# YihongSun/Dynamo-Depth

Hardware: AMD Instinct MI355X
Metric: training images/sec (192x640 triplets) (higher is better)
Workload: dtype f32

## Files before the change

dynamo-depth_amd/csrc/dd_conv_mfma.hip:

```cpp
#include <hip/hip_runtime.h>
#include <cstdlib>
#include <type_traits>

#include "../../include/dynamo_hip.h"
#include "dd_attr.h"
#include "dd_split.h"
#include "dd_store_tile.h"

namespace dd {
namespace cm {

constexpr int TH = 8, TW = 32, NT = 256;
constexpr int HH = TH + 2, HW = TW + 2, HN = HH * HW;
constexpr int CK = 16;
constexpr int PSTR = 48;
constexpr int A_PIECE = HN * PSTR;
constexpr int A_BYTES = 3 * A_PIECE;
__device__ __forceinline__ int halo_addr(int px, int half) {
  return px * 48 + half * 16;
}
__host__ __device__ constexpr int pieces_of(int products) { return products == 6 ? 3 : (products == 3 ? 2 : 1); }
constexpr int FRAG = 1024;
constexpr int PRE = (HN * 4 + NT - 1) / NT;

__host__ __device__ inline int blocks_for(int n_out) { return n_out <= 32 ? 1 : (n_out <= 64 ? 2 : (n_out <= 96 ? 3 : 2)); }
__host__ __device__ inline int frags_of(int n_out, int k_in) {
  const int NB = blocks_for(n_out);
  return ((n_out + 32 * NB - 1) / (32 * NB)) * ((k_in + CK - 1) / CK) * 9 * NB;
}

template <int NB>
constexpr int b_buf_bytes() { return ((3 * NB + 3) / 4) * 4 * FRAG; }

template <int NB>
constexpr int lds_bytes() { return A_BYTES + 2 * b_buf_bytes<NB>(); }

__device__ __forceinline__ void pack_fragment(const float* __restrict__ w, long long s_co, long long s_ci, long long s_kh, long long s_kw, int cout, int cin,
                                              uint4* __restrict__ pack_fwd, uint4* __restrict__ pack_bwd, int frags_fwd, int frags_bwd, int gid) {
  const int lane = gid & 63;
  int f = gid >> 6;
  const bool bwd = f >= frags_fwd;
  if (bwd) f -= frags_fwd;
  if (bwd ? (f >= frags_bwd || !pack_bwd) : !pack_fwd) return;
  const int n_out = bwd ? cin : cout, k_in = bwd ? cout : cin;
  const int nchunks = (k_in + CK - 1) / CK, NB = blocks_for(n_out);
  const int blk = f % NB, tap = (f / NB) % 9, chunk = (f / (NB * 9)) % nchunks, tile = f / (NB * 9 * nchunks);
  const int o = (tile * NB + blk) * 32 + (lane & 31);
  const int i0 = chunk * CK + (lane >> 5) * 8;
  const int kh = tap / 3, kw = tap % 3;
  float v[8];
#pragma unroll
  for (int e = 0; e < 8; ++e) {
    const int i = i0 + e;
    float val = 0.f;
    if (o < n_out && i < k_in)
      val = bwd ? w[(long long)i * s_co + (long long)o * s_ci + (2 - kh) * s_kh + (2 - kw) * s_kw]
                : w[(long long)o * s_co + (long long)i * s_ci + kh * s_kh + kw * s_kw];
    v[e] = val;
  }
  unsigned p[3][4];
#pragma unroll
  for (int q = 0; q < 4; ++q) split2(v[2 * q], v[2 * q + 1], p[0][q], p[1][q], p[2][q]);
  uint4* dst = (bwd ? pack_bwd : pack_fwd) + ((size_t)f * 3) * 64 + lane;
#pragma unroll
  for (int pc = 0; pc < 3; ++pc) dst[pc * 64] = make_uint4(p[pc][0], p[pc][1], p[pc][2], p[pc][3]);
}

__global__ __launch_bounds__(256) void conv_mfma_pack_kernel(const float* __restrict__ w, long long s_co, long long s_ci, long long s_kh, long long s_kw,
                                                             int cout, int cin, uint4* __restrict__ pack_fwd, uint4* __restrict__ pack_bwd,
                                                             int frags_fwd, int frags_bwd) {
  pack_fragment(w, s_co, s_ci, s_kh, s_kw, cout, cin, pack_fwd, pack_bwd, frags_fwd, frags_bwd, blockIdx.x * 256 + threadIdx.x);
}

constexpr int PACK_JOB_WORDS = 10;
__global__ __launch_bounds__(256) void conv_mfma_pack_many_kernel(const long long* __restrict__ jobs, const int* __restrict__ block_job) {
  const long long* j = jobs + (size_t)block_job[blockIdx.x] * PACK_JOB_WORDS;
  const int cout = (int)j[5], cin = (int)j[6];
  uint4* const pf = reinterpret_cast<uint4*>(j[7]);
  uint4* const pb = reinterpret_cast<uint4*>(j[8]);
  const int frags_fwd = pf ? frags_of(cout, cin) : 0, frags_bwd = pb ? frags_of(cin, cout) : 0;
  pack_fragment(reinterpret_cast<const float*>(j[0]), j[1], j[2], j[3], j[4], cout, cin, pf, pb, frags_fwd, frags_bwd,
                (blockIdx.x - (int)j[9]) * 256 + threadIdx.x);
}

template <int NB, int NP>
__global__ __launch_bounds__(NT, 2) void conv_mfma_kernel(const float* __restrict__ x, const uint4* __restrict__ pack, const float* __restrict__ bias,
                                                          int Hi, int Wi, int Ho, int Wo, int k_in, int n_out, int pad, int tiles_x, int tiles_y,
                                                          float* __restrict__ y) {
  extern __shared__ __align__(16) unsigned char smem[];
  unsigned char* const s_b = smem + A_BYTES;
  const int tid = threadIdx.x, lane = tid & 63, wave = __builtin_amdgcn_readfirstlane(tid >> 6);
  const int b = blockIdx.z, ntile = blockIdx.y;
  int tile = blockIdx.x;
  {
    const int ntiles = gridDim.x, xc = tile & 7, base = ntiles >> 3, extra = ntiles & 7;
    tile = xc * base + min(xc, extra) + (tile >> 3);
  }
  const int X0 = (tile % tiles_x) * TW, Y0 = (tile / tiles_x) * TH;
  const int nchunks = (k_in + CK - 1) / CK;
  const float* xb = x + (size_t)b * Hi * Wi * k_in;
  const char* pk = reinterpret_cast<const char*>(pack) + (size_t)ntile * nchunks * 9 * (3 * NB * FRAG);

  int g_off[PRE];
  int l_off[PRE];
#pragma unroll
  for (int j = 0; j < PRE; ++j) {
    const int i = tid + j * NT, px = i >> 2, q = i & 3;
    const int hy = px / HW, hx = px - hy * HW;
    const int Y = Y0 - pad + hy, X = X0 - pad + hx;
    l_off[j] = px < HN ? halo_addr(px, q >> 1) + (q & 1) * 8 : -1;
    g_off[j] = (px < HN && Y >= 0 && Y < Hi && X >= 0 && X < Wi) ? (Y * Wi + X) * k_in + q * 4 : -1;
  }
  float4 pre[PRE];
  auto fetch = [&](int chunk) {
#pragma unroll
    for (int j = 0; j < PRE; ++j) {
      const int c0 = chunk * CK + (((tid + j * NT) & 3) << 2);
      const int off = (g_off[j] >= 0 && c0 < k_in) ? g_off[j] + chunk * CK : 0;
      pre[j] = *reinterpret_cast<const float4*>(xb + off);
    }
  };
  auto stage = [&](int chunk) {
#pragma unroll
    for (int j = 0; j < PRE; ++j) {
      if (l_off[j] >= 0) {
        const int c0 = chunk * CK + (((tid + j * NT) & 3) << 2);
        const bool in = g_off[j] >= 0 && c0 < k_in;
        const float4 v = in ? pre[j] : make_float4(0.f, 0.f, 0.f, 0.f);
        unsigned a1, a2, a3, b1, b2, b3;
        split2(v.x, v.y, a1, a2, a3);
        split2(v.z, v.w, b1, b2, b3);
        *reinterpret_cast<uint2*>(smem + l_off[j]) = make_uint2(a1, b1);
        if (pieces_of(NP) > 1) *reinterpret_cast<uint2*>(smem + A_PIECE + l_off[j]) = make_uint2(a2, b2);
        if (pieces_of(NP) > 2) *reinterpret_cast<uint2*>(smem + 2 * A_PIECE + l_off[j]) = make_uint2(a3, b3);
      }
    }
  };
  constexpr int BR = (3 * NB + 3) / 4;
  uint4 breg[BR];
#pragma unroll
  for (int r = 0; r < BR; ++r) breg[r] = make_uint4(0u, 0u, 0u, 0u);
  auto fetch_b = [&](int s) {
    const char* src = pk + (size_t)s * (3 * NB * FRAG) + lane * 16;
#pragma unroll
    for (int r = 0; r < BR; ++r)
      breg[r] = *reinterpret_cast<const uint4*>(src + (wave + 4 * r < 3 * NB ? wave + 4 * r : 0) * FRAG);
  };
  auto store_b = [&](int s) {
    unsigned char* dst = s_b + (s & 1) * b_buf_bytes<NB>() + lane * 16;
#pragma unroll
    for (int r = 0; r < BR; ++r) *reinterpret_cast<uint4*>(dst + (wave + 4 * r) * FRAG) = breg[r];
  };
  auto lds_barrier = [&]() { asm volatile("s_waitcnt lgkmcnt(0)\n\ts_barrier" ::: "memory"); };

  f16v acc[2][NB];
#pragma unroll
  for (int m = 0; m < 2; ++m)
#pragma unroll
    for (int n = 0; n < NB; ++n)
#pragma unroll
      for (int r = 0; r < 16; ++r) acc[m][n][r] = 0.f;

  const int a_pix = (2 * wave) * HW + (lane & 31), a_half = lane >> 5;
  const unsigned char* b_lane = s_b + lane * 16;

  uint4 af[2][2][3], bfr[2][NB][3];
  auto read_frags = [&](int set, int tap, int s) {
    const int ty = tap / 3, tx = tap % 3;
#pragma unroll
    for (int m = 0; m < 2; ++m) {
      const unsigned char* ap = smem + halo_addr(a_pix + (m + ty) * HW + tx, a_half);
#pragma unroll
      for (int pc = 0; pc < pieces_of(NP); ++pc) af[set][m][pc] = *reinterpret_cast<const uint4*>(ap + pc * A_PIECE);
    }
    const unsigned char* bb = b_lane + (s & 1) * b_buf_bytes<NB>();
#pragma unroll
    for (int n = 0; n < NB; ++n)
#pragma unroll
      for (int pc = 0; pc < pieces_of(NP); ++pc) bfr[set][n][pc] = *reinterpret_cast<const uint4*>(bb + (n * 3 + pc) * FRAG);
  };

  const int nsteps = nchunks * 9;
  float bv[NB];
#pragma unroll
  for (int n = 0; n < NB; ++n) bv[n] = tile_bias(bias, (ntile * NB + n) * 32 + (lane & 31), n_out, pack);
  fetch_b(0);
  fetch(0);
  store_b(0);
  fetch_b(1);
  for (int chunk = 0; chunk < nchunks; ++chunk) {
    lds_barrier();
    stage(chunk);
    store_b(chunk * 9 + 1);
    lds_barrier();
    read_frags(0, 0, chunk * 9);
#pragma unroll
    for (int tap = 0; tap < 9; ++tap) {
      const int s = chunk * 9 + tap, cur = tap & 1;
      if (tap < 8) read_frags(cur ^ 1, tap + 1, s + 1);
      fetch_b(min(s + 2, nsteps - 1));
      if (tap == 1) fetch(min(chunk + 1, nchunks - 1));
      constexpr int PA[6] = {2, 0, 1, 1, 0, 0}, PB[6] = {0, 2, 1, 0, 1, 0};
#pragma unroll
      for (int t = 6 - NP; t < 6; ++t)
#pragma unroll
        for (int m = 0; m < 2; ++m)
#pragma unroll
          for (int n = 0; n < NB; ++n)
            acc[m][n] = __builtin_amdgcn_mfma_f32_32x32x16_bf16(__builtin_bit_cast(bf8, af[cur][m][PA[t]]), __builtin_bit_cast(bf8, bfr[cur][n][PB[t]]), acc[m][n], 0, 0, 0);
      __builtin_amdgcn_sched_barrier(0);
      if (tap < 8) {
        store_b(s + 2);
        lds_barrier();
      }
    }
  }

  auto tail = [&](auto full) {
#pragma unroll
    for (int n = 0; n < NB; ++n) {
      const int co = (ntile * NB + n) * 32 + (lane & 31);
#pragma unroll
      for (int m = 0; m < 2; ++m) {
        const int Y = Y0 + 2 * wave + m, X = X0 + 4 * (lane >> 5);
        float* p = y + (((size_t)b * Ho + Y) * Wo + X) * n_out + co;
        store_acc32<decltype(full)::value>(acc[m][n], bv[n], p, (size_t)n_out, (co < n_out && Y < Ho) ? Wo - X : 0, StoreF32{});
      }
    }
  };
  if (X0 + TW <= Wo && Y0 + TH <= Ho && (ntile + 1) * (32 * NB) <= n_out) tail(std::true_type{});
  else tail(std::false_type{});
}

constexpr int FLAT_MT = 256;
constexpr int FLAT_ZERO = HN - 1;
constexpr int FLAT_MAX_W = (FLAT_ZERO - FLAT_MT) / 2 - 1;

template <int NB, int NP>
__global__ __launch_bounds__(NT, 2) void conv_mfma_flat_kernel(const float* __restrict__ x, const uint4* __restrict__ pack, const float* __restrict__ bias,
                                                               int H, int W, int M, int k_in, int n_out, int splits, float* __restrict__ out) {
  extern __shared__ __align__(16) unsigned char smem[];
  unsigned char* const s_b = smem + A_BYTES;
  const int tid = threadIdx.x, lane = tid & 63, wave = __builtin_amdgcn_readfirstlane(tid >> 6);
  const int p0 = (int)blockIdx.x * FLAT_MT, ntile = blockIdx.y, split = blockIdx.z;
  const int nchunks = (k_in + CK - 1) / CK;
  const int c_begin = (int)((long long)nchunks * split / splits), c_end = (int)((long long)nchunks * (split + 1) / splits);
  const int win = FLAT_MT + 2 * (W + 1), q0 = p0 - (W + 1);
  const char* pk = reinterpret_cast<const char*>(pack) + (size_t)ntile * nchunks * 9 * (3 * NB * FRAG);

  int g_off[PRE], l_off[PRE];
#pragma unroll
  for (int j = 0; j < PRE; ++j) {
    const int i = tid + j * NT, px = i >> 2, q = i & 3;
    const int fp = q0 + px;
    l_off[j] = px < win ? halo_addr(px, q >> 1) + (q & 1) * 8 : -1;
    g_off[j] = (px < win && fp >= 0 && fp < M) ? fp * k_in + q * 4 : -1;
  }
  if (tid < 9) {
    const int pc = tid / 3, part = tid % 3;
    if (part * 16 < PSTR) *reinterpret_cast<uint4*>(smem + pc * A_PIECE + FLAT_ZERO * PSTR + part * 16) = make_uint4(0u, 0u, 0u, 0u);
  }
  float4 pre[PRE];
  auto fetch = [&](int chunk) {
#pragma unroll
    for (int j = 0; j < PRE; ++j) {
      const int c0 = chunk * CK + (((tid + j * NT) & 3) << 2);
      const int off = (g_off[j] >= 0 && c0 < k_in) ? g_off[j] + chunk * CK : 0;
      pre[j] = *reinterpret_cast<const float4*>(x + off);
    }
  };
  auto stage = [&](int chunk) {
#pragma unroll
    for (int j = 0; j < PRE; ++j) {
      if (l_off[j] >= 0) {
        const int c0 = chunk * CK + (((tid + j * NT) & 3) << 2);
        const bool in = g_off[j] >= 0 && c0 < k_in;
        const float4 v = in ? pre[j] : make_float4(0.f, 0.f, 0.f, 0.f);
        unsigned a1, a2, a3, b1, b2, b3;
        split2(v.x, v.y, a1, a2, a3);
        split2(v.z, v.w, b1, b2, b3);
        *reinterpret_cast<uint2*>(smem + l_off[j]) = make_uint2(a1, b1);
        if (pieces_of(NP) > 1) *reinterpret_cast<uint2*>(smem + A_PIECE + l_off[j]) = make_uint2(a2, b2);
        if (pieces_of(NP) > 2) *reinterpret_cast<uint2*>(smem + 2 * A_PIECE + l_off[j]) = make_uint2(a3, b3);
      }
    }
  };
  constexpr int BR = (3 * NB + 3) / 4;
  uint4 breg[BR];
#pragma unroll
  for (int r = 0; r < BR; ++r) breg[r] = make_uint4(0u, 0u, 0u, 0u);
  auto fetch_b = [&](int s) {
    const char* src = pk + (size_t)s * (3 * NB * FRAG) + lane * 16;
#pragma unroll
    for (int r = 0; r < BR; ++r) breg[r] = *reinterpret_cast<const uint4*>(src + (wave + 4 * r < 3 * NB ? wave + 4 * r : 0) * FRAG);
  };
  auto store_b = [&](int s) {
    unsigned char* dst = s_b + (s & 1) * b_buf_bytes<NB>() + lane * 16;
#pragma unroll
    for (int r = 0; r < BR; ++r) *reinterpret_cast<uint4*>(dst + (wave + 4 * r) * FRAG) = breg[r];
  };
  auto lds_barrier = [&]() { asm volatile("s_waitcnt lgkmcnt(0)\n\ts_barrier" ::: "memory"); };

  f16v acc[2][NB];
#pragma unroll
  for (int m = 0; m < 2; ++m)
#pragma unroll
    for (int n = 0; n < NB; ++n)
#pragma unroll
      for (int r = 0; r < 16; ++r) acc[m][n][r] = 0.f;

  unsigned tapmask[2];
  int a_base[2];
#pragma unroll
  for (int m = 0; m < 2; ++m) {
    const int loc = (2 * wave + m) * 32 + (lane & 31), p = p0 + loc;
    const int rem = p % (H * W), yy = rem / W, xx = rem - yy * W;
    unsigned mk = 0u;
#pragma unroll
    for (int t = 0; t < 9; ++t) {
      const int Y = yy + t / 3 - 1, X = xx + t % 3 - 1;
      if (p < M && Y >= 0 && Y < H && X >= 0 && X < W) mk |= 1u << t;
    }
    tapmask[m] = mk;
    a_base[m] = (W + 1) + loc;
  }
  const unsigned char* b_lane = s_b + lane * 16;

  uint4 af[2][2][3], bfr[2][NB][3];
  auto read_frags = [&](int set, int tap, int s) {
    const int toff = (tap / 3 - 1) * W + (tap % 3 - 1);
#pragma unroll
    for (int m = 0; m < 2; ++m) {
      const int addr = halo_addr(((tapmask[m] >> tap) & 1u) ? a_base[m] + toff : FLAT_ZERO, lane >> 5);
#pragma unroll
      for (int pc = 0; pc < pieces_of(NP); ++pc) af[set][m][pc] = *reinterpret_cast<const uint4*>(smem + addr + pc * A_PIECE);
    }
    const unsigned char* bb = b_lane + (s & 1) * b_buf_bytes<NB>();
#pragma unroll
    for (int n = 0; n < NB; ++n)
#pragma unroll
      for (int pc = 0; pc < pieces_of(NP); ++pc) bfr[set][n][pc] = *reinterpret_cast<const uint4*>(bb + (n * 3 + pc) * FRAG);
  };

  const int s_last = c_end * 9 - 1;
  float bv[NB];
#pragma unroll
  for (int n = 0; n < NB; ++n) bv[n] = tile_bias(splits == 1 ? bias : nullptr, (ntile * NB + n) * 32 + (lane & 31), n_out, pack);
  fetch_b(c_begin * 9);
  fetch(c_begin);
  store_b(c_begin * 9);
  fetch_b(min(c_begin * 9 + 1, s_last));
  for (int chunk = c_begin; chunk < c_end; ++chunk) {
    lds_barrier();
    stage(chunk);
    store_b(chunk * 9 + 1);
    lds_barrier();
    read_frags(0, 0, chunk * 9);
#pragma unroll
    for (int tap = 0; tap < 9; ++tap) {
      const int s = chunk * 9 + tap, cur = tap & 1;
      if (tap < 8) read_frags(cur ^ 1, tap + 1, s + 1);
      fetch_b(min(s + 2, s_last));
      if (tap == 1) fetch(min(chunk + 1, c_end - 1));
      constexpr int PA[6] = {2, 0, 1, 1, 0, 0}, PB[6] = {0, 2, 1, 0, 1, 0};
#pragma unroll
      for (int t = 6 - NP; t < 6; ++t)
#pragma unroll
        for (int m = 0; m < 2; ++m)
#pragma unroll
          for (int n = 0; n < NB; ++n)
            acc[m][n] = __builtin_amdgcn_mfma_f32_32x32x16_bf16(__builtin_bit_cast(bf8, af[cur][m][PA[t]]), __builtin_bit_cast(bf8, bfr[cur][n][PB[t]]), acc[m][n], 0, 0, 0);
      __builtin_amdgcn_sched_barrier(0);
      if (tap < 8) {
        store_b(s + 2);
        lds_barrier();
      }
    }
  }

  float* dst = out + (splits > 1 ? (size_t)split * M * n_out : 0);
  auto tail = [&](auto full) {
#pragma unroll
    for (int n = 0; n < NB; ++n) {
      const int co = (ntile * NB + n) * 32 + (lane & 31);
#pragma unroll
      for (int m = 0; m < 2; ++m) {
        const int p = p0 + (2 * wave + m) * 32 + 4 * (lane >> 5);
        store_acc32<decltype(full)::value>(acc[m][n], bv[n], dst + (size_t)p * n_out + co, (size_t)n_out, co < n_out ? M - p : 0, StoreF32{});
      }
    }
  };
  if (p0 + FLAT_MT <= M && (ntile + 1) * (32 * NB) <= n_out) tail(std::true_type{});
  else tail(std::false_type{});
}

__global__ __launch_bounds__(256) void conv_flat_fold_kernel(const float* __restrict__ part, const float* __restrict__ bias, int total4, int n_out, int splits,
                                                             float* __restrict__ y) {
  const int i = blockIdx.x * 256 + threadIdx.x;
  if (i >= total4) return;
  const float4* P = reinterpret_cast<const float4*>(part);
  float4 a = P[i];
  for (int s = 1; s < splits; ++s) {
    const float4 v = P[(size_t)s * total4 + i];
    a.x += v.x; a.y += v.y; a.z += v.z; a.w += v.w;
  }
  if (bias) {
    const int c = (i * 4) % n_out;
    a.x += bias[c]; a.y += bias[c + 1]; a.z += bias[c + 2]; a.w += bias[c + 3];
  }
  reinterpret_cast<float4*>(y)[i] = a;
}

static int flat_splits(int M, int k_in, int n_out) {
  const int wgs = ((M + FLAT_MT - 1) / FLAT_MT) * ((n_out + 63) / 64), nchunks = (k_in + CK - 1) / CK;
  const char* env = getenv("DD_FLAT_SPLITS");
  int s = env ? atoi(env) : (480 + wgs / 2) / wgs;
  if (s > nchunks / 2) s = nchunks / 2;
  return s < 1 ? 1 : s;
}

static size_t pack_bytes(int n_out, int k_in) { return (size_t)frags_of(n_out, k_in) * 3 * FRAG; }

template <int NB, int NP>
static int launch(const float* x, const void* pack, const float* bias, int B, int Hi, int Wi, int k_in, int n_out, int pad, float* y, hipStream_t stream) {
  const int Ho = Hi + 2 * pad - 2, Wo = Wi + 2 * pad - 2;
  const int tiles_x = (Wo + TW - 1) / TW, tiles_y = (Ho + TH - 1) / TH;
  auto kern = conv_mfma_kernel<NB, NP>;
  static dd::LdsAttrOnce lds_attr;
  if (const int rc = lds_attr.ensure(reinterpret_cast<const void*>(kern), (int)(lds_bytes<NB>()))) return rc;
  dim3 grid(tiles_x * tiles_y, (n_out + 32 * NB - 1) / (32 * NB), B);
  hipLaunchKernelGGL(kern, grid, dim3(NT), lds_bytes<NB>(), stream, x, static_cast<const uint4*>(pack), bias, Hi, Wi, Ho, Wo, k_in, n_out, pad, tiles_x,
                     tiles_y, y);
  return (int)hipGetLastError();
}

template <int NP>
static int launch_blocks(const float* x, const void* pack, const float* bias, int B, int Hi, int Wi, int k_in, int n_out, int pad, float* y, hipStream_t s) {
  switch (blocks_for(n_out)) {
    case 1: return launch<1, NP>(x, pack, bias, B, Hi, Wi, k_in, n_out, pad, y, s);
    case 2: return launch<2, NP>(x, pack, bias, B, Hi, Wi, k_in, n_out, pad, y, s);
    default: return launch<3, NP>(x, pack, bias, B, Hi, Wi, k_in, n_out, pad, y, s);
  }
}

template <int NP>
static int launch_flat(const float* x, const void* pack, const float* bias, int H, int W, int M, int k_in, int n_out, int splits, float* out, hipStream_t s) {
  auto kern = conv_mfma_flat_kernel<2, NP>;
  static dd::LdsAttrOnce lds_attr;
  if (const int rc = lds_attr.ensure(reinterpret_cast<const void*>(kern), (int)(lds_bytes<2>()))) return rc;
  hipLaunchKernelGGL(kern, dim3((M + FLAT_MT - 1) / FLAT_MT, (n_out + 63) / 64, splits), dim3(NT), lds_bytes<2>(), s, x, static_cast<const uint4*>(pack), bias, H, W, M, k_in,
                     n_out, splits, out);
  return (int)hipGetLastError();
}

namespace wg {
constexpr int TR = 2, TC = 16;
constexpr int XR = TR + 2, XC = TC + 2;
constexpr int XROW = 24;
constexpr int GSTR = TR * TC * 2 + 16;
constexpr int XSTR = XR * XROW * 2 + 16;
constexpr int G_PIECE = 64 * GSTR, X_PIECE = 64 * XSTR;
constexpr int LDS = 3 * (G_PIECE + X_PIECE);
constexpr int XITEMS = XR * (XC / 2) * 16;
constexpr int XJ = (XITEMS + NT - 1) / NT;
constexpr int BLOCK = 64 * 9 * 64;
}

template <int NP>
__global__ __launch_bounds__(NT, 2) void conv_wgrad_kernel(const float* __restrict__ x, const float* __restrict__ g, int B, int Hi, int Wi, int Ho, int Wo,
                                                           int cin, int cout, int pad, int tiles_x, int tiles_y, float* __restrict__ partial) {
  using namespace wg;
  extern __shared__ __align__(16) unsigned char smem[];
  unsigned char* const s_g = smem;
  unsigned char* const s_x = smem + 3 * G_PIECE;
  const int tid = threadIdx.x, lane = tid & 63, wave = __builtin_amdgcn_readfirstlane(tid >> 6);
  const int ks = blockIdx.x, nks = gridDim.x, ci0 = blockIdx.y * 64, co0 = blockIdx.z * 64;
  const int total = B * tiles_y * tiles_x;
  const int t_begin = (int)((long long)total * ks / nks), t_end = (int)((long long)total * (ks + 1) / nks);

  const int gq = tid >> 4, grow = (tid >> 3) & 1, gpair = tid & 7;
  const int g_lds = (4 * gq) * GSTR + (grow * TC + 2 * gpair) * 2;
  int xq[XJ], xrow[XJ], xpair[XJ], x_lds[XJ];
#pragma unroll
  for (int j = 0; j < XJ; ++j) {
    const int item = tid + j * NT;
    xq[j] = item / (XR * (XC / 2));
    const int rem = item - xq[j] * (XR * (XC / 2));
    xrow[j] = rem / (XC / 2);
    xpair[j] = rem - xrow[j] * (XC / 2);
    x_lds[j] = item < XITEMS ? (4 * xq[j]) * XSTR + (xrow[j] * XROW + 2 * xpair[j]) * 2 : -1;
  }
  const bool g_ch = co0 + 4 * gq < cout;

  float4 pg[2], px[XJ][2];
  auto fetch = [&](int t) {
    const int b = t / (tiles_y * tiles_x), r = t - b * (tiles_y * tiles_x);
    const int Y0 = (r / tiles_x) * TR, X0 = (r - (r / tiles_x) * tiles_x) * TC;
    {
      const int Y = Y0 + grow, X = X0 + 2 * gpair;
      const float* src = g + (((size_t)b * Ho + Y) * Wo + X) * cout + co0 + 4 * gq;
      const bool ok = g_ch && Y < Ho;
      pg[0] = (ok && X < Wo) ? *reinterpret_cast<const float4*>(src) : make_float4(0.f, 0.f, 0.f, 0.f);
      pg[1] = (ok && X + 1 < Wo) ? *reinterpret_cast<const float4*>(src + cout) : make_float4(0.f, 0.f, 0.f, 0.f);
    }
#pragma unroll
    for (int j = 0; j < XJ; ++j) {
      const int Y = Y0 - pad + xrow[j], X = X0 - pad + 2 * xpair[j];
      const bool ok = x_lds[j] >= 0 && ci0 + 4 * xq[j] < cin && Y >= 0 && Y < Hi;
      const float* src = x + (((ptrdiff_t)b * Hi + Y) * Wi + X) * cin + ci0 + 4 * xq[j];
      px[j][0] = (ok && X >= 0 && X < Wi) ? *reinterpret_cast<const float4*>(src) : make_float4(0.f, 0.f, 0.f, 0.f);
      px[j][1] = (ok && X + 1 >= 0 && X + 1 < Wi) ? *reinterpret_cast<const float4*>(src + cin) : make_float4(0.f, 0.f, 0.f, 0.f);
    }
  };
  auto put = [&](unsigned char* plane, int piece_bytes, int stride, int off, const float4& a, const float4& b) {
    const float av[4] = {a.x, a.y, a.z, a.w}, bv[4] = {b.x, b.y, b.z, b.w};
#pragma unroll
    for (int c = 0; c < 4; ++c) {
      unsigned p1, p2, p3;
      split2(av[c], bv[c], p1, p2, p3);
      *reinterpret_cast<unsigned*>(plane + off + c * stride) = p1;
      if (pieces_of(NP) > 1) *reinterpret_cast<unsigned*>(plane + piece_bytes + off + c * stride) = p2;
      if (pieces_of(NP) > 2) *reinterpret_cast<unsigned*>(plane + 2 * piece_bytes + off + c * stride) = p3;
    }
  };
  auto stage = [&]() {
    put(s_g, G_PIECE, GSTR, g_lds, pg[0], pg[1]);
#pragma unroll
    for (int j = 0; j < XJ; ++j)
      if (x_lds[j] >= 0) put(s_x, X_PIECE, XSTR, x_lds[j], px[j][0], px[j][1]);
  };

  const int ngroups = (cin - ci0 > 32) ? 6 : 3;
  const int g_full = wave, g_half = 4 + (wave >> 1), half = wave & 1;
  const bool full_on = g_full < ngroups, half_on = g_half < ngroups;
  auto group_off = [&](int g) { return (g / 3) * 32 * XSTR + (g % 3) * (XROW * 2); };
  const int off_full = group_off(g_full), off_half = group_off(g_half);
  f16v acc[9];
#pragma unroll
  for (int a = 0; a < 9; ++a)
#pragma unroll
    for (int r = 0; r < 16; ++r) acc[a][r] = 0.f;

  const unsigned char* a_lane = s_g + (lane & 31) * GSTR + (lane >> 5) * 16;
  const unsigned char* b_lane = s_x + (lane & 31) * XSTR + (lane >> 5) * 16;
  constexpr int PA[6] = {2, 0, 1, 1, 0, 0}, PB[6] = {0, 2, 1, 0, 1, 0};
  auto shifted = [](const uint4& w0, unsigned w1, int tx) -> uint4 {
    if (tx == 0) return w0;
    if (tx == 2) return make_uint4(w0.y, w0.z, w0.w, w1);
    return make_uint4(__builtin_amdgcn_alignbit(w0.y, w0.x, 16), __builtin_amdgcn_alignbit(w0.z, w0.y, 16), __builtin_amdgcn_alignbit(w0.w, w0.z, 16),
                      __builtin_amdgcn_alignbit(w1, w0.w, 16));
  };

  if (t_begin < t_end) fetch(t_begin);
  for (int t = t_begin; t < t_end; ++t) {
    __syncthreads();
    stage();
    __syncthreads();
    if (t + 1 < t_end) fetch(t + 1);
#pragma unroll
    for (int row = 0; row < TR; ++row) {
      uint4 af[2][3];
#pragma unroll
      for (int m = 0; m < 2; ++m)
#pragma unroll
        for (int pc = 0; pc < pieces_of(NP); ++pc) af[m][pc] = *reinterpret_cast<const uint4*>(a_lane + m * 32 * GSTR + row * (TC * 2) + pc * G_PIECE);
      uint4 w0[3];
      unsigned w1[3];
      if (full_on) {
#pragma unroll
        for (int pc = 0; pc < pieces_of(NP); ++pc) {
          const unsigned char* src = b_lane + off_full + row * (XROW * 2) + pc * X_PIECE;
          w0[pc] = *reinterpret_cast<const uint4*>(src);
          w1[pc] = *reinterpret_cast<const unsigned*>(src + 16);
        }
#pragma unroll
        for (int tx = 0; tx < 3; ++tx) {
          uint4 bf[3];
#pragma unroll
          for (int pc = 0; pc < pieces_of(NP); ++pc) bf[pc] = shifted(w0[pc], w1[pc], tx);
#pragma unroll
          for (int tt = 6 - NP; tt < 6; ++tt)
#pragma unroll
            for (int m = 0; m < 2; ++m)
              acc[tx * 2 + m] = __builtin_amdgcn_mfma_f32_32x32x16_bf16(__builtin_bit_cast(bf8, af[m][PA[tt]]), __builtin_bit_cast(bf8, bf[PB[tt]]),
                                                                        acc[tx * 2 + m], 0, 0, 0);
          __builtin_amdgcn_sched_barrier(0);
        }
      }
      if (half_on) {
#pragma unroll
        for (int pc = 0; pc < pieces_of(NP); ++pc) {
          const unsigned char* src = b_lane + off_half + row * (XROW * 2) + pc * X_PIECE;
          w0[pc] = *reinterpret_cast<const uint4*>(src);
          w1[pc] = *reinterpret_cast<const unsigned*>(src + 16);
        }
        {
          const int txd = half == 0 ? 0 : 2;
          uint4 bf[3];
#pragma unroll
          for (int pc = 0; pc < pieces_of(NP); ++pc) bf[pc] = txd == 0 ? shifted(w0[pc], w1[pc], 0) : shifted(w0[pc], w1[pc], 2);
#pragma unroll
          for (int tt = 6 - NP; tt < 6; ++tt)
#pragma unroll
            for (int m = 0; m < 2; ++m)
              acc[6 + m] = __builtin_amdgcn_mfma_f32_32x32x16_bf16(__builtin_bit_cast(bf8, af[m][PA[tt]]), __builtin_bit_cast(bf8, bf[PB[tt]]), acc[6 + m], 0, 0, 0);
          __builtin_amdgcn_sched_barrier(0);
          uint4 am[3];
#pragma unroll
          for (int pc = 0; pc < pieces_of(NP); ++pc) {
            bf[pc] = shifted(w0[pc], w1[pc], 1);
            am[pc] = half == 0 ? af[0][pc] : af[1][pc];
          }
#pragma unroll
          for (int tt = 6 - NP; tt < 6; ++tt)
            acc[8] = __builtin_amdgcn_mfma_f32_32x32x16_bf16(__builtin_bit_cast(bf8, am[PA[tt]]), __builtin_bit_cast(bf8, bf[PB[tt]]), acc[8], 0, 0, 0);
        }
      }
    }
  }

  float* P = partial + (((size_t)blockIdx.z * gridDim.y + blockIdx.y) * nks + ks) * BLOCK;
  auto put_acc = [&](const f16v& A, int g, int tx, int m) {
    const int nb = g / 3, tap = (g % 3) * 3 + tx;
#pragma unroll
    for (int r = 0; r < 16; ++r) {
      const int co = m * 32 + (r & 3) + 8 * (r >> 2) + 4 * (lane >> 5);
      P[(co * 9 + tap) * 64 + nb * 32 + (lane & 31)] = A[r];
    }
  };
  if (full_on) {
#pragma unroll
    for (int tx = 0; tx < 3; ++tx)
#pragma unroll
      for (int m = 0; m < 2; ++m) put_acc(acc[tx * 2 + m], g_full, tx, m);
  }
  if (half_on) {
    put_acc(acc[6], g_half, half == 0 ? 0 : 2, 0);
    put_acc(acc[7], g_half, half == 0 ? 0 : 2, 1);
    put_acc(acc[8], g_half, 1, half);
  }
}

__global__ __launch_bounds__(256) void conv_wgrad_fold_kernel(const float* __restrict__ partial, int nks, int cin, int cout, int ci_groups, float* __restrict__ gw) {
  __shared__ float red[4][64];
  const int lane = threadIdx.x & 63, wave = threadIdx.x >> 6;
  const int idx = blockIdx.x * 64 + lane;
  const bool in = idx < cout * 9 * cin;
  float s[8] = {0.f, 0.f, 0.f, 0.f, 0.f, 0.f, 0.f, 0.f};
  if (in) {
    const int ci = idx % cin, tap = (idx / cin) % 9, co = idx / (9 * cin);
    const int z = co >> 6, y = ci >> 6;
    const float* P = partial + ((size_t)z * ci_groups + y) * nks * wg::BLOCK + ((co & 63) * 9 + tap) * 64 + (ci & 63);
    int k = wave;
    for (; k + 28 < nks; k += 32) {
#pragma unroll
      for (int j = 0; j < 8; ++j) s[j] += P[(size_t)(k + 4 * j) * wg::BLOCK];
    }
    for (; k < nks; k += 4) s[0] += P[(size_t)k * wg::BLOCK];
  }
  red[wave][lane] = ((s[0] + s[1]) + (s[2] + s[3])) + ((s[4] + s[5]) + (s[6] + s[7]));
  __syncthreads();
  if (wave == 0 && in) gw[idx] = (red[0][lane] + red[1][lane]) + (red[2][lane] + red[3][lane]);
}

static int wgrad_splits(int B, int Ho, int Wo, int cin, int cout) {
  const int groups = ((cin + 63) / 64) * ((cout + 63) / 64);
  const int tiles = B * ((Ho + wg::TR - 1) / wg::TR) * ((Wo + wg::TC - 1) / wg::TC);
  int n = 512 / groups;
  if (n > tiles / 11) n = tiles / 11;
  return n < 1 ? 1 : n;
}

}
}

extern "C" int dd_conv3x3_mfma_supported(int cin, int cout) {
  return (cin >= 16 && cout >= 16 && cin % 4 == 0 && cout % 4 == 0 && cin <= 1024 && cout <= 1024) ? 1 : 0;
}

extern "C" size_t dd_conv3x3_mfma_pack_bytes(int n_out, int k_in) { return dd::cm::pack_bytes(n_out, k_in); }

extern "C" int dd_conv3x3_mfma_pack(const float* weight, long long s_co, long long s_ci, long long s_kh, long long s_kw, int cout, int cin, void* pack_fwd,
                                    void* pack_bwd_data, void* stream) {
  using namespace dd::cm;
  if (!weight || (!pack_fwd && !pack_bwd_data) || cout < 1 || cin < 1) return (int)hipErrorInvalidValue;
  const int frags_fwd = pack_fwd ? (int)(pack_bytes(cout, cin) / (3 * FRAG)) : 0;
  const int frags_bwd = pack_bwd_data ? (int)(pack_bytes(cin, cout) / (3 * FRAG)) : 0;
  const int threads = (frags_fwd + frags_bwd) * 64;
  hipLaunchKernelGGL(conv_mfma_pack_kernel, dim3((threads + 255) / 256), dim3(256), 0, static_cast<hipStream_t>(stream), weight, s_co, s_ci, s_kh, s_kw, cout,
                     cin, static_cast<uint4*>(pack_fwd), static_cast<uint4*>(pack_bwd_data), frags_fwd, frags_bwd);
  return (int)hipGetLastError();
}

extern "C" int dd_conv3x3_mfma_pack_many_job_words(void) { return dd::cm::PACK_JOB_WORDS; }

extern "C" int dd_conv3x3_mfma_pack_many_blocks(int cout, int cin, int want_fwd, int want_bwd_data) {
  using namespace dd::cm;
  if (cout < 1 || cin < 1) return 0;
  return ((want_fwd ? frags_of(cout, cin) : 0) + (want_bwd_data ? frags_of(cin, cout) : 0) + 3) / 4;
}

extern "C" int dd_conv3x3_mfma_pack_many(const long long* jobs, const int* block_job, int n_blocks, void* stream) {
  using namespace dd::cm;
  if (!jobs || !block_job || n_blocks < 1) return (int)hipErrorInvalidValue;
  hipLaunchKernelGGL(conv_mfma_pack_many_kernel, dim3(n_blocks), dim3(256), 0, static_cast<hipStream_t>(stream), jobs, block_job);
  return (int)hipGetLastError();
}

extern "C" int dd_conv3x3_mfma_n(const float* x, const void* pack, const float* bias, int B, int Hi, int Wi, int k_in, int n_out, int pad, int products,
                                 float* y, void* stream) {
  using namespace dd::cm;
  if (!x || !pack || !y || B < 1 || pad < 0 || pad > 2 || Hi + 2 * pad < 3 || Wi + 2 * pad < 3 || k_in % 4 || k_in < 4 || n_out < 1) return (int)hipErrorInvalidValue;
  if ((size_t)Hi * Wi * k_in >= (1ull << 31) || (reinterpret_cast<unsigned long long>(x) & 15ull)) return (int)hipErrorInvalidValue;
  hipStream_t s = static_cast<hipStream_t>(stream);
  switch (products) {
    case 6: return launch_blocks<6>(x, pack, bias, B, Hi, Wi, k_in, n_out, pad, y, s);
    case 3: return launch_blocks<3>(x, pack, bias, B, Hi, Wi, k_in, n_out, pad, y, s);
    case 1: return launch_blocks<1>(x, pack, bias, B, Hi, Wi, k_in, n_out, pad, y, s);
    default: return (int)hipErrorInvalidValue;
  }
}

extern "C" int dd_conv3x3_mfma(const float* x, const void* pack, const float* bias, int B, int Hi, int Wi, int k_in, int n_out, int pad, float* y,
                               void* stream) {
  return dd_conv3x3_mfma_n(x, pack, bias, B, Hi, Wi, k_in, n_out, pad, 6, y, stream);
}

extern "C" int dd_conv3x3_mfma_flat_supported(int B, int H, int W, int k_in, int n_out) {
  using namespace dd::cm;
  return (B >= 1 && H >= 1 && W >= 1 && W <= FLAT_MAX_W && k_in >= 32 && k_in % 4 == 0 && k_in <= 1024 && n_out % 4 == 0 && n_out <= 1024 &&
          blocks_for(n_out) == 2 && n_out > 32 &&
          (size_t)B * H * W * (size_t)(k_in > n_out ? k_in : n_out) < (1ull << 31)) ? 1 : 0;
}

extern "C" size_t dd_conv3x3_mfma_flat_workspace_bytes(int B, int H, int W, int k_in, int n_out) {
  using namespace dd::cm;
  const int M = B * H * W, s = flat_splits(M, k_in, n_out);
  return s > 1 ? (size_t)s * M * n_out * sizeof(float) : 16;
}

extern "C" int dd_conv3x3_mfma_flat_n(const float* x, const void* pack, const float* bias, int B, int H, int W, int k_in, int n_out, int products, float* y,
                                      void* workspace, size_t workspace_bytes, void* stream) {
  using namespace dd::cm;
  if (!x || !pack || !y || !dd_conv3x3_mfma_flat_supported(B, H, W, k_in, n_out) || (reinterpret_cast<unsigned long long>(x) & 15ull) ||
      (reinterpret_cast<unsigned long long>(y) & 15ull) || (products != 6 && products != 3 && products != 1))
    return (int)hipErrorInvalidValue;
  const int M = B * H * W, splits = flat_splits(M, k_in, n_out);
  if (splits > 1 && (!workspace || workspace_bytes < dd_conv3x3_mfma_flat_workspace_bytes(B, H, W, k_in, n_out) || (reinterpret_cast<unsigned long long>(workspace) & 15ull)))
    return (int)hipErrorInvalidValue;
  hipStream_t s = static_cast<hipStream_t>(stream);
  float* out = splits > 1 ? static_cast<float*>(workspace) : y;
  const int rc = products == 6 ? launch_flat<6>(x, pack, bias, H, W, M, k_in, n_out, splits, out, s)
               : products == 3 ? launch_flat<3>(x, pack, bias, H, W, M, k_in, n_out, splits, out, s)
                               : launch_flat<1>(x, pack, bias, H, W, M, k_in, n_out, splits, out, s);
  if (rc != 0 || splits == 1) return rc;
  const int total4 = M * n_out / 4;
  hipLaunchKernelGGL(conv_flat_fold_kernel, dim3((total4 + 255) / 256), dim3(256), 0, s, static_cast<const float*>(workspace), bias, total4, n_out, splits, y);
  return (int)hipGetLastError();
}

extern "C" int dd_conv3x3_mfma_flat(const float* x, const void* pack, const float* bias, int B, int H, int W, int k_in, int n_out, float* y, void* workspace,
                                    size_t workspace_bytes, void* stream) {
  return dd_conv3x3_mfma_flat_n(x, pack, bias, B, H, W, k_in, n_out, 6, y, workspace, workspace_bytes, stream);
}

extern "C" size_t dd_conv3x3_mfma_wgrad_workspace_bytes(int B, int Ho, int Wo, int cin, int cout) {
  const size_t groups = (size_t)((cin + 63) / 64) * ((cout + 63) / 64);
  return groups * dd::cm::wgrad_splits(B, Ho, Wo, cin, cout) * dd::cm::wg::BLOCK * sizeof(float);
}

extern "C" int dd_conv3x3_mfma_bwd_weight_n(const float* x, const float* g_out, int B, int Hi, int Wi, int cin, int cout, int pad, int products, float* g_weight,
                                            void* workspace, size_t workspace_bytes, void* stream) {
  using namespace dd::cm;
  if (!x || !g_out || !g_weight || !workspace || B < 1 || pad < 0 || pad > 1 || cin % 4 || cout % 4 || cin < 4 || cout < 4) return (int)hipErrorInvalidValue;
  if (products != 6 && products != 3 && products != 1) return (int)hipErrorInvalidValue;
  const int Ho = Hi + 2 * pad - 2, Wo = Wi + 2 * pad - 2;
  if (Ho < 1 || Wo < 1 || workspace_bytes < dd_conv3x3_mfma_wgrad_workspace_bytes(B, Ho, Wo, cin, cout)) return (int)hipErrorInvalidValue;
  if ((size_t)B * Hi * Wi * cin >= (1ull << 31) || (size_t)B * Ho * Wo * cout >= (1ull << 31)) return (int)hipErrorInvalidValue;
  if ((reinterpret_cast<unsigned long long>(x) | reinterpret_cast<unsigned long long>(g_out)) & 15ull) return (int)hipErrorInvalidValue;
  hipStream_t s = static_cast<hipStream_t>(stream);
  const int tiles_x = (Wo + wg::TC - 1) / wg::TC, tiles_y = (Ho + wg::TR - 1) / wg::TR;
  const int nks = wgrad_splits(B, Ho, Wo, cin, cout), ci_groups = (cin + 63) / 64, co_groups = (cout + 63) / 64;
  const dim3 grid(nks, ci_groups, co_groups);
  float* part = static_cast<float*>(workspace);
  if (products == 6)
    hipLaunchKernelGGL(conv_wgrad_kernel<6>, grid, dim3(NT), wg::LDS, s, x, g_out, B, Hi, Wi, Ho, Wo, cin, cout, pad, tiles_x, tiles_y, part);
  else if (products == 3)
    hipLaunchKernelGGL(conv_wgrad_kernel<3>, grid, dim3(NT), wg::LDS, s, x, g_out, B, Hi, Wi, Ho, Wo, cin, cout, pad, tiles_x, tiles_y, part);
  else
    hipLaunchKernelGGL(conv_wgrad_kernel<1>, grid, dim3(NT), wg::LDS, s, x, g_out, B, Hi, Wi, Ho, Wo, cin, cout, pad, tiles_x, tiles_y, part);
  hipError_t e = hipGetLastError();
  if (e != hipSuccess) return (int)e;
  hipLaunchKernelGGL(conv_wgrad_fold_kernel, dim3((cout * 9 * cin + 63) / 64), dim3(256), 0, s, static_cast<const float*>(workspace), nks, cin, cout, ci_groups,
                     g_weight);
  return (int)hipGetLastError();
}

extern "C" int dd_conv3x3_mfma_bwd_weight(const float* x, const float* g_out, int B, int Hi, int Wi, int cin, int cout, int pad, float* g_weight, void* workspace,
                                          size_t workspace_bytes, void* stream) {
  return dd_conv3x3_mfma_bwd_weight_n(x, g_out, B, Hi, Wi, cin, cout, pad, 6, g_weight, workspace, workspace_bytes, stream);
}
```

Before: 355.8.

## Add warp-specialized producer/consumer MFMA conv kernel for small grids

Adds a 512-thread conv kernel in which four loader waves stage the input halo (split into bf16 pieces) and weight fragments into double-buffered and ring LDS buffers, while four compute waves run the MFMA taps. Blocks can process a run of tiles persistently, with a tile remap that spreads work across XCDs. By default it is used only when the tile count fits within the CU count (run length 1), aiming to hide global-load latency behind MFMA work on small layers. It doubles LDS use for A and adds a per-tap barrier, which may lower occupancy.

```diff
diff --git a/dynamo-depth_amd/csrc/dd_conv_mfma.hip b/dynamo-depth_amd/csrc/dd_conv_mfma.hip
--- a/dynamo-depth_amd/csrc/dd_conv_mfma.hip
+++ b/dynamo-depth_amd/csrc/dd_conv_mfma.hip
@@ -232,6 +232,248 @@
   else tail(std::false_type{});
 }
 
+constexpr int NT2 = 512, RING = 4;
+
+template <int NB>
+constexpr int lw_lds_bytes() { return 2 * A_BYTES + RING * b_buf_bytes<NB>(); }
+
+template <int NB, int NP>
+__global__ __launch_bounds__(NT2) void conv_mfma_lw_kernel(const float* __restrict__ x, const uint4* __restrict__ pack, const float* __restrict__ bias, int Hi,
+                                                           int Wi, int Ho, int Wo, int k_in, int n_out, int pad, int tiles_x, int tiles_xy, int ntn, int total,
+                                                           int run, float* __restrict__ y) {
+  extern __shared__ __align__(16) unsigned char smem[];
+  unsigned char* const s_b = smem + 2 * A_BYTES;
+  const int tid = threadIdx.x, lane = tid & 63, wave = __builtin_amdgcn_readfirstlane(tid >> 6);
+  const int nchunks = (k_in + CK - 1) / CK, nsteps = nchunks * 9;
+  const int L0 = blockIdx.x * run;
+  const int ntl = min(run, total - L0), Q = ntl * nchunks;
+  constexpr int STEP_BYTES = 3 * NB * FRAG;
+  auto tile_of = [&](int L, int& b, int& ntile, int& X0, int& Y0) {
+    const int raw = L % tiles_xy, rest = L / tiles_xy;
+    ntile = rest % ntn;
+    b = rest / ntn;
+    const int xc = raw & 7, base = tiles_xy >> 3, extra = tiles_xy & 7;
+    const int tile = xc * base + min(xc, extra) + (raw >> 3);
+    X0 = (tile % tiles_x) * TW;
+    Y0 = (tile / tiles_x) * TH;
+  };
+  auto lds_barrier = [&]() { asm volatile("s_waitcnt lgkmcnt(0)\n\ts_barrier" ::: "memory"); };
+
+  if (wave >= 4) {
+    const int lt = tid - 4 * 64, lw = wave - 4;
+    int l_off[PRE], g_off[PRE];
+#pragma unroll
+    for (int j = 0; j < PRE; ++j) {
+      const int i = lt + j * NT, px = i >> 2, q = i & 3;
+      l_off[j] = px < HN ? halo_addr(px, q >> 1) + (q & 1) * 8 : -1;
+    }
+    const float* xb = x;
+    auto set_tile = [&](int L) {
+      int b, ntile, X0, Y0;
+      tile_of(L, b, ntile, X0, Y0);
+      xb = x + (size_t)b * Hi * Wi * k_in;
+#pragma unroll
+      for (int j = 0; j < PRE; ++j) {
+        const int i = lt + j * NT, px = i >> 2, q = i & 3;
+        const int hy = px / HW, hx = px - hy * HW;
+        const int Y = Y0 - pad + hy, X = X0 - pad + hx;
+        g_off[j] = (px < HN && Y >= 0 && Y < Hi && X >= 0 && X < Wi) ? (Y * Wi + X) * k_in + q * 4 : -1;
+      }
+    };
+    int f_q = 0, f_chunk = 0, f_tile = 0, p_chunk = 0;
+    float4 pre[PRE];
+    auto fetch = [&]() {
+      p_chunk = f_chunk;
+#pragma unroll
+      for (int j = 0; j < PRE; ++j) {
+        const int c0 = f_chunk * CK + (((lt + j * NT) & 3) << 2);
+        const int off = (g_off[j] >= 0 && c0 < k_in) ? g_off[j] + f_chunk * CK : 0;
+        pre[j] = *reinterpret_cast<const float4*>(xb + off);
+      }
+    };
+    auto advance = [&]() {
+      if (f_q + 1 < Q) {
+        ++f_q;
+        if (++f_chunk == nchunks) {
+          f_chunk = 0;
+          ++f_tile;
+          set_tile(L0 + f_tile);
+        }
+      }
+    };
+    auto stage_one = [&](int j, unsigned char* hb) {
+      if (l_off[j] >= 0) {
+        const int c0 = p_chunk * CK + (((lt + j * NT) & 3) << 2);
+        const bool in = g_off[j] >= 0 && c0 < k_in;
+        const float4 v = in ? pre[j] : make_float4(0.f, 0.f, 0.f, 0.f);
+        unsigned a1, a2, a3, b1, b2, b3;
+        split2(v.x, v.y, a1, a2, a3);
+        split2(v.z, v.w, b1, b2, b3);
+        *reinterpret_cast<uint2*>(hb + l_off[j]) = make_uint2(a1, b1);
+        if (pieces_of(NP) > 1) *reinterpret_cast<uint2*>(hb + A_PIECE + l_off[j]) = make_uint2(a2, b2);
+        if (pieces_of(NP) > 2) *reinterpret_cast<uint2*>(hb + 2 * A_PIECE + l_off[j]) = make_uint2(a3, b3);
+      }
+    };
+    constexpr int BR = (3 * NB + 3) / 4;
+    int b_s = 0, b_tile = 0;
+    auto pack_of = [&](int L) { return reinterpret_cast<const char*>(pack) + (size_t)((L / tiles_xy) % ntn) * nsteps * STEP_BYTES; };
+    const char* pk = pack_of(L0);
+    struct BRegs { uint4 v[BR]; };
+    auto fetch_b = [&]() {
+      const char* src = pk + (size_t)b_s * STEP_BYTES + lane * 16;
+      BRegs r;
+#pragma unroll
+      for (int k = 0; k < BR; ++k) r.v[k] = *reinterpret_cast<const uint4*>(src + (lw + 4 * k < 3 * NB ? lw + 4 * k : 0) * FRAG);
+      if (b_s + 1 < nsteps) {
+        ++b_s;
+      } else if (b_tile + 1 < ntl) {
+        ++b_tile;
+        b_s = 0;
+        pk = pack_of(L0 + b_tile);
+      }
+      return r;
+    };
+    auto store_b = [&](const BRegs& r, int slot) {
+      unsigned char* dst = s_b + slot * b_buf_bytes<NB>() + lane * 16;
+#pragma unroll
+      for (int k = 0; k < BR; ++k) *reinterpret_cast<uint4*>(dst + (lw + 4 * k) * FRAG) = r.v[k];
+    };
+
+    set_tile(L0);
+    BRegs breg[3];
+#pragma unroll
+    for (int k = 0; k < 3; ++k) breg[k] = fetch_b();
+    fetch();
+#pragma unroll
+    for (int k = 0; k < 3; ++k) store_b(breg[k], k);
+#pragma unroll
+    for (int k = 0; k < 3; ++k) breg[k] = fetch_b();
+#pragma unroll
+    for (int j = 0; j < PRE; ++j) stage_one(j, smem);
+    advance();
+    fetch();
+    lds_barrier();
+    int G = 0;
+    for (int q = 0; q < Q; ++q) {
+      unsigned char* const hb = smem + ((q + 1) & 1) * A_BYTES;
+#pragma unroll
+      for (int tap = 0; tap < 9; ++tap) {
+        if (tap >= 1 && tap <= PRE) stage_one(tap - 1, hb);
+        store_b(breg[tap % 3], (G + 3) & 3);
+        breg[tap % 3] = fetch_b();
+        if (tap == PRE) {
+          advance();
+          fetch();
+        }
+        lds_barrier();
+        ++G;
+      }
+    }
+    return;
+  }
+
+  const int a_lane = halo_addr((2 * wave) * HW + (lane & 31), lane >> 5);
+  const unsigned char* b_lane = s_b + lane * 16;
+  uint4 af[2][2][3], bfr[2][NB][3];
+  auto read_frags = [&](auto setc, int pc0, int pc1, int tap, const unsigned char* hbuf, int slot) {
+    constexpr int set = decltype(setc)::value;
+    const int ty = tap / 3, tx = tap % 3;
+#pragma unroll
+    for (int m = 0; m < 2; ++m) {
+      const unsigned char* ap = hbuf + a_lane + halo_addr((m + ty) * HW + tx, 0);
+#pragma unroll
+      for (int pc = pc0; pc < pc1; ++pc) af[set][m][pc] = *reinterpret_cast<const uint4*>(ap + pc * A_PIECE);
+    }
+    const unsigned char* bb = b_lane + slot * b_buf_bytes<NB>();
+#pragma unroll
+    for (int n = 0; n < NB; ++n)
+#pragma unroll
+      for (int pc = pc0; pc < pc1; ++pc) bfr[set][n][pc] = *reinterpret_cast<const uint4*>(bb + (n * 3 + pc) * FRAG);
+  };
+  f16v acc[2][NB];
+  int q = 0, G = 0;
+  auto chunk_body = [&]() {
+    const unsigned char* const h_cur = smem + (q & 1) * A_BYTES;
+    const unsigned char* const h_nxt = smem + ((q + 1) & 1) * A_BYTES;
+#pragma unroll
+    for (int tap = 0; tap < 9; ++tap) {
+      constexpr int PA[6] = {2, 0, 1, 1, 0, 0}, PB[6] = {0, 2, 1, 0, 1, 0};
+      const int cur = tap & 1, slot = (G + 1) & 3;
+      const int ntap = tap < 8 ? tap + 1 : 0;
+      const unsigned char* const h = tap < 8 ? h_cur : h_nxt;
+      constexpr int EARLY = pieces_of(NP) < 2 ? pieces_of(NP) : 2;
+      if (cur) read_frags(std::integral_constant<int, 0>{}, 0, EARLY, ntap, h, slot);
+      else read_frags(std::integral_constant<int, 1>{}, 0, EARLY, ntap, h, slot);
+      __builtin_amdgcn_sched_barrier(0);
+#pragma unroll
+      for (int t = 6 - NP; t < 6; ++t) {
+        if (t == 2 && NP == 6) {
+          __builtin_amdgcn_sched_barrier(0);
+          if (cur) read_frags(std::integral_constant<int, 0>{}, 2, 3, ntap, h, slot);
+          else read_frags(std::integral_constant<int, 1>{}, 2, 3, ntap, h, slot);
+          __builtin_amdgcn_sched_barrier(0);
+        }
+#pragma unroll
+        for (int m = 0; m < 2; ++m)
+#pragma unroll
+          for (int n = 0; n < NB; ++n)
+            acc[m][n] = __builtin_amdgcn_mfma_f32_32x32x16_bf16(__builtin_bit_cast(bf8, af[cur][m][PA[t]]), __builtin_bit_cast(bf8, bfr[cur][n][PB[t]]), acc[m][n], 0, 0, 0);
+      }
+      __builtin_amdgcn_sched_barrier(0);
+      lds_barrier();
+      ++G;
+    }
+#pragma unroll
+    for (int pc = 0; pc < 3; ++pc) {
+#pragma unroll
+      for (int m = 0; m < 2; ++m) af[0][m][pc] = af[1][m][pc];
+#pragma unroll
+      for (int n = 0; n < NB; ++n) bfr[0][n][pc] = bfr[1][n][pc];
+    }
+  };
+
+  int b, ntile, X0, Y0;
+  tile_of(L0, b, ntile, X0, Y0);
+  float bv[NB];
+#pragma unroll
+  for (int n = 0; n < NB; ++n) bv[n] = tile_bias(bias, (ntile * NB + n) * 32 + (lane & 31), n_out, pack);
+  lds_barrier();
+  read_frags(std::integral_constant<int, 0>{}, 0, pieces_of(NP), 0, smem, 0);
+  for (int ti = 0; ti < ntl; ++ti) {
+    if (ti > 0) {
+      tile_of(L0 + ti, b, ntile, X0, Y0);
+#pragma unroll
+      for (int n = 0; n < NB; ++n) bv[n] = tile_bias(bias, (ntile * NB + n) * 32 + (lane & 31), n_out, pack);
+    }
+#pragma unroll
+    for (int m = 0; m < 2; ++m)
+#pragma unroll
+      for (int n = 0; n < NB; ++n)
+#pragma unroll
+        for (int r = 0; r < 16; ++r) acc[m][n][r] = 0.f;
+    for (int c = 0; c < nchunks; ++c) {
+      chunk_body();
+      ++q;
+    }
+#pragma unroll
+    for (int n = 0; n < NB; ++n) asm volatile("" : "+v"(bv[n]));
+    auto tail = [&](auto full) {
+#pragma unroll
+      for (int n = 0; n < NB; ++n) {
+        const int co = (ntile * NB + n) * 32 + (lane & 31);
+#pragma unroll
+        for (int m = 0; m < 2; ++m) {
+          const int Y = Y0 + 2 * wave + m, X = X0 + 4 * (lane >> 5);
+          float* p = y + (((size_t)b * Ho + Y) * Wo + X) * n_out + co;
+          store_acc32<decltype(full)::value>(acc[m][n], bv[n], p, (size_t)n_out, (co < n_out && Y < Ho) ? Wo - X : 0, StoreF32{});
+        }
+      }
+    };
+    if (X0 + TW <= Wo && Y0 + TH <= Ho && (ntile + 1) * (32 * NB) <= n_out) tail(std::true_type{});
+    else tail(std::false_type{});
+  }
+}
+
 constexpr int FLAT_MT = 256;
 constexpr int FLAT_ZERO = HN - 1;
 constexpr int FLAT_MAX_W = (FLAT_ZERO - FLAT_MT) / 2 - 1;
@@ -421,10 +663,41 @@
 
 static size_t pack_bytes(int n_out, int k_in) { return (size_t)frags_of(n_out, k_in) * 3 * FRAG; }
 
+static int cu_count() {
+  static std::atomic<int> cached[64];
+  int dev = 0;
+  if (hipGetDevice(&dev) != hipSuccess) return 256;
+  std::atomic<int>& c = cached[dev & 63];
+  int n = c.load(std::memory_order_relaxed);
+  if (n <= 0) {
+    if (hipDeviceGetAttribute(&n, hipDeviceAttributeMultiprocessorCount, dev) != hipSuccess || n <= 0) n = 256;
+    c.store(n, std::memory_order_relaxed);
+  }
+  return n;
+}
+
+static int run_length(int total) {
+  const char* env = getenv("DD_CONV_MFMA_RUN");
+  if (!env) return total <= cu_count() ? 1 : 0;
+  const int r = atoi(env);
+  return r <= 0 ? 0 : (r > total ? total : r);
+}
+
 template <int NB, int NP>
 static int launch(const float* x, const void* pack, const float* bias, int B, int Hi, int Wi, int k_in, int n_out, int pad, float* y, hipStream_t stream) {
   const int Ho = Hi + 2 * pad - 2, Wo = Wi + 2 * pad - 2;
   const int tiles_x = (Wo + TW - 1) / TW, tiles_y = (Ho + TH - 1) / TH;
+  const int ntn = (n_out + 32 * NB - 1) / (32 * NB);
+  const long long total = (long long)tiles_x * tiles_y * ntn * B;
+  const int run = total < (1ll << 30) ? run_length((int)total) : 0;
+  if (run > 0) {
+    auto lw = conv_mfma_lw_kernel<NB, NP>;
+    static dd::LdsAttrOnce lw_attr;
+    if (const int rc = lw_attr.ensure(reinterpret_cast<const void*>(lw), (int)(lw_lds_bytes<NB>()))) return rc;
+    hipLaunchKernelGGL(lw, dim3(((int)total + run - 1) / run), dim3(NT2), lw_lds_bytes<NB>(), stream, x, static_cast<const uint4*>(pack), bias, Hi, Wi, Ho, Wo, k_in,
+                       n_out, pad, tiles_x, tiles_x * tiles_y, ntn, (int)total, run, y);
+    return (int)hipGetLastError();
+  }
   auto kern = conv_mfma_kernel<NB, NP>;
   static dd::LdsAttrOnce lds_attr;
   if (const int rc = lds_attr.ensure(reinterpret_cast<const void*>(kern), (int)(lds_bytes<NB>()))) return rc;
```

Measured after the change: 354.9. No clear change (-0.2%).
